# chargen/ALCHEMY

Measured on AMD Instinct MI355X. Metric: ctxt-mul+relinearize/sec at n=2^15, 4 RNS limbs, higher is better.
Workload: dtype u32; 1 GPU; BASELINE config 3: keySwitchQuadCirc(hint, a*b) on linear ciphertexts, n=2^15 (m'=2^16), L=4 primes<2^31, TrivGad hint at the same modulus, CRT-basis in/out, inputs resident in HBM; batch_per_gpu=8192, global_batch=8192, hint=single rank, device_word_bytes=4

## Files before the change

alchemy_amd/csrc/kernel_tensor_split.hpp:

```cpp
#pragma once
#include <hip/hip_runtime.h>
#include "ntt_engine.hpp"

#ifndef ALCH_TI_SPLIT_PASSES
#define ALCH_TI_SPLIT_PASSES 4
#endif

#ifndef ALCH_TI_NT_IN
#define ALCH_TI_NT_IN 0
#endif

#ifndef ALCH_A_PARTIALS
#define ALCH_A_PARTIALS 0
#endif

namespace alch {

template <int LOGN, bool Q30 = false>
__global__ void __launch_bounds__(1 << (LOGN - 6), 4)
k_tensor_intt_split(DevRing<u32> R, const u32* __restrict__ a, const u32* __restrict__ b, int32_t* __restrict__ digits,
                    unsigned nitems, Scal<u32> spre
#if ALCH_A_PARTIALS
                    , const u32* __restrict__ hint, u32* __restrict__ out
#endif
                    ) {
    typedef u32 W;
    constexpr int LOGM = LOGN - 1, M = 1 << LOGM, LT = LOGN - 6, T = 1 << LT;
    typedef Geo<LOGM, LT> G;
    static_assert(G::E == 32 && (LOGM - 2) % 4 == 0, "32 coefficients per lane, stages 4+4+4+2");
    typedef u32 V __attribute__((ext_vector_type(4)));
    typedef int32_t SV __attribute__((ext_vector_type(4)));
    constexpr int NV = G::E / 4;
    extern __shared__ __attribute__((aligned(16))) unsigned char smem[];
    W* lds = reinterpret_cast<W*>(smem);
    const int L = R.L;
    const u32 nct = nitems / (unsigned)L;
    const auto ra = __builtin_amdgcn_make_buffer_rsrc(const_cast<W*>(a), 0, (u32)((size_t)nct * 2 * L * (2 * M) * 4), 0x00020000);
    const auto rb = __builtin_amdgcn_make_buffer_rsrc(const_cast<W*>(b), 0, (u32)((size_t)nct * 2 * L * (2 * M) * 4), 0x00020000);
    const auto rd = __builtin_amdgcn_make_buffer_rsrc(digits, 0, (u32)((size_t)nct * L * (2 * M) * 4), 0x00020000);
    const u32 lane16 = threadIdx.x * 16u;
    constexpr u32 ROW = (u32)(2 * M) * 4u, SLICE = (u32)T * 16u, HALF = (u32)M * 4u;
#if ALCH_A_PARTIALS
    const auto rh = __builtin_amdgcn_make_buffer_rsrc(const_cast<W*>(hint), 0, (u32)((size_t)2 * L * L * (2 * M) * 4), 0x00020000);
    const auto ro = __builtin_amdgcn_make_buffer_rsrc(out, 0, (u32)((size_t)nct * 2 * L * (2 * M) * 4), 0x00020000);
#endif

    for (unsigned item = blockIdx.x; item < nitems; item += gridDim.x) {
        const u32 ct = item / (unsigned)L, i = item % (unsigned)L;
        const ModP<W> m = R.mod[i];
        const W q = m.q, qni = m.qni;
        const W ninv_s = mont_mul(R.ninv_m[i], spre.v[i], m), w1ninv_s = mont_mul(R.w1ninv_m[i], spre.v[i], m);
        const u32 row = ((2 * ct + 1) * (u32)L + i) * ROW;
        const u32 drow = (ct * (u32)L + i) * ROW;
        const int rot = (int)((item ^ (item >> 3)) & (NV - 1));
        const W* twi = R.twi[i];
        V keep[NV];
#pragma unroll 1
        for (int half = 0; half < 2; ++half) {
            int tid = threadIdx.x;
            asm volatile("" : "+v"(tid));
#pragma unroll
            for (int r = 0; r < NV; ++r) {
                const u32 so = row + (u32)half * HALF + SLICE * (u32)((r + rot) & (NV - 1));
                const V va = __builtin_bit_cast(V, __builtin_amdgcn_raw_buffer_load_b128(ra, lane16, so, ALCH_TI_NT_IN));
                const V vb = __builtin_bit_cast(V, __builtin_amdgcn_raw_buffer_load_b128(rb, lane16, so, ALCH_TI_NT_IN));
#if ALCH_A_PARTIALS
                if (out) {
                    const u32 so0 = so - (u32)L * ROW;
                    const u32 piece = (u32)half * HALF + SLICE * (u32)((r + rot) & (NV - 1));
                    const u32 hrow = ((2 * i) * (u32)L + i) * ROW + piece;
                    const V a0v = __builtin_bit_cast(V, __builtin_amdgcn_raw_buffer_load_b128(ra, lane16, so0, ALCH_TI_NT_IN));
                    const V b0v = __builtin_bit_cast(V, __builtin_amdgcn_raw_buffer_load_b128(rb, lane16, so0, ALCH_TI_NT_IN));
                    const V h0v = __builtin_bit_cast(V, __builtin_amdgcn_raw_buffer_load_b128(rh, lane16, hrow, 0));
                    const V h1v = __builtin_bit_cast(V, __builtin_amdgcn_raw_buffer_load_b128(rh, lane16, hrow + (u32)L * ROW, 0));
                    const W sr2 = spre.v[i];
                    V o0v, o1v;
#pragma unroll
                    for (int e = 0; e < 4; ++e) {
                        const W x0 = csub(mont_mul_lazy(a0v[e], sr2, q, qni), q);
                        const W x1 = csub(mont_mul_lazy(va[e], sr2, q, qni), q);
                        const W c2 = csub(mont_mul_lazy(vb[e], x1, q, qni), q);
                        const u64 p0 = (u64)x0 * b0v[e] + (u64)c2 * h0v[e];
                        const u32 m0 = (u32)p0 * qni;
                        o0v[e] = csub((u32)((p0 + (u64)m0 * q) >> 32), q);
                        const u64 p1 = (u64)x0 * vb[e] + (u64)x1 * b0v[e] + (u64)c2 * h1v[e];
                        const u64 p1r = ((u64)csub((W)(p1 >> 32), q) << 32) | (u32)p1;
                        const u32 m1 = (u32)p1r * qni;
                        o1v[e] = csub((u32)((p1r + (u64)m1 * q) >> 32), q);
                    }
                    __builtin_amdgcn_raw_buffer_store_b128(__builtin_bit_cast(decltype(__builtin_amdgcn_raw_buffer_load_b128(ro, 0, 0, 0)), o0v), ro, lane16, so0, 0);
                    ALCH_STORE_GUARD(o0v);
                    __builtin_amdgcn_raw_buffer_store_b128(__builtin_bit_cast(decltype(__builtin_amdgcn_raw_buffer_load_b128(ro, 0, 0, 0)), o1v), ro, lane16, so, 0);
                    ALCH_STORE_GUARD(o1v);
                }
#endif
                V v;
#pragma unroll
                for (int e = 0; e < 4; ++e) v[e] = mont_mul_lazy(va[e], vb[e], q, qni);
                *reinterpret_cast<V*>(&lds[swz<LOGM>((tid + T * ((r + rot) & (NV - 1))) * 4)]) = v;
            }
            lds_barrier();
            NoEpilogue none;
            const int prefix = 2 + half;
#if ALCH_TI_SPLIT_PASSES == 3
            ntt_pass<LOGM, LT, W, 9, 5, true, false, false, W, NoEpilogue&, false, Q30>(lds, twi, q, qni, (W)0, (W)0, tid, prefix, none);
            lds_barrier();
            ntt_pass<LOGM, LT, W, 4, 5, true, false, false, W, NoEpilogue&, false, Q30>(lds, twi, q, qni, (W)0, (W)0, tid, prefix, none);
            lds_barrier();
            ntt_pass<LOGM, LT, W, 0, 4, true, false, false, W, NoEpilogue&, false, Q30>(lds, twi, q, qni, (W)0, (W)0, tid, prefix, none);
            lds_barrier();
#else
            ntt_pass<LOGM, LT, W, 10, 4, true, false, false, W, NoEpilogue&, false, Q30>(lds, twi, q, qni, (W)0, (W)0, tid, prefix, none);
            pair_sync<LOGM>();
            ntt_pass<LOGM, LT, W, 6, 4, true, false, false, W, NoEpilogue&, false, Q30>(lds, twi, q, qni, (W)0, (W)0, tid, prefix, none);
            lds_barrier();
            ntt_pass<LOGM, LT, W, 2, 4, true, false, false, W, NoEpilogue&, false, Q30>(lds, twi, q, qni, (W)0, (W)0, tid, prefix, none);
            lds_barrier();
            ntt_pass<LOGM, LT, W, 0, 2, true, false, false, W, NoEpilogue&, false, Q30>(lds, twi, q, qni, (W)0, (W)0, tid, prefix, none);
            lds_barrier();
#endif
            if (half == 0) {
#pragma unroll
                for (int r = 0; r < NV; ++r) keep[r] = *reinterpret_cast<const V*>(&lds[swz<LOGM>((tid + T * r) * 4)]);
            } else {
                const W hq = (q - 1) >> 1;
#pragma unroll
                for (int r = 0; r < NV; ++r) {
                    const V hi = *reinterpret_cast<const V*>(&lds[swz<LOGM>((tid + T * r) * 4)]);
                    SV z0, z1;
#pragma unroll
                    for (int e = 0; e < 4; ++e) {
                        const W x = csub(keep[r][e], q), y = csub(hi[e], q);
                        const W c0 = csub(mont_mul_lazy((W)(x + y), ninv_s, q, qni), q);
                        const W c1 = csub(mont_mul_lazy((W)(x - y + q), w1ninv_s, q, qni), q);
                        z0[e] = c0 > hq ? (int32_t)c0 - (int32_t)q : (int32_t)c0;
                        z1[e] = c1 > hq ? (int32_t)c1 - (int32_t)q : (int32_t)c1;
                    }
                    const u32 so = drow + SLICE * (u32)r;
                    __builtin_amdgcn_raw_buffer_store_b128(__builtin_bit_cast(decltype(__builtin_amdgcn_raw_buffer_load_b128(rd, 0, 0, 0)), z0), rd, lane16, so, 0);
                    ALCH_STORE_GUARD(z0);
                    __builtin_amdgcn_raw_buffer_store_b128(__builtin_bit_cast(decltype(__builtin_amdgcn_raw_buffer_load_b128(rd, 0, 0, 0)), z1), rd, lane16, so + HALF, 0);
                    ALCH_STORE_GUARD(z1);
                }
            }
            lds_barrier();
        }
    }
}

}
```

alchemy_amd/csrc/ntt_engine.hpp:

```cpp
#pragma once
#include "modarith.hpp"

namespace alch {

template <int LOGN, int LOGT_ = -1>
struct Geo {
    static_assert(LOGN >= 4 && LOGN <= 15, "ring dimension 16 .. 32768 per LDS-resident transform");
    static constexpr int N = 1 << LOGN;
    static constexpr int LOGT = LOGT_ >= 0 ? LOGT_ : ((LOGN - 4 > 10) ? 10 : (LOGN - 4));
    static constexpr int T = 1 << LOGT;
    static constexpr int E = N / T;
    static constexpr int NPASS = (LOGN + 3) / 4;
    static constexpr int NS0 = LOGN - 4 * (NPASS - 1);
    static constexpr bool SWZ = LOGN >= 10;
};

#ifndef ALCH_LDS_PAD
#define ALCH_LDS_PAD 1
#endif
template <int LOGN>
__host__ __device__ constexpr int swz(int idx) {
#if ALCH_LDS_PAD
    return (LOGN >= 10) ? idx + ((idx >> 6) << 2) : idx;
#else
    return (LOGN >= 10) ? (idx ^ (((idx >> 6) & 3) << 2) ^ (((idx >> 8) & 3) << 4)) : idx;
#endif
}
__host__ __device__ constexpr int lds_join(int mapped_base, int mapped_k) {
#if ALCH_LDS_PAD
    return mapped_base + mapped_k;
#else
    return mapped_base ^ mapped_k;
#endif
}
template <int LOGN>
__host__ __device__ constexpr int lds_words() {
#if ALCH_LDS_PAD
    return (LOGN >= 10) ? (1 << LOGN) + (1 << (LOGN - 4)) : (1 << LOGN);
#else
    return 1 << LOGN;
#endif
}

template <typename W> struct Vec4;
template <> struct Vec4<u32> { typedef u32 type __attribute__((ext_vector_type(4))); static constexpr int LANES = 4; };
template <> struct Vec4<u64> { typedef u64 type __attribute__((ext_vector_type(2))); static constexpr int LANES = 2; };

#ifndef ALCH_NO_STORE_GUARD
#define ALCH_STORE_GUARD(v) asm volatile("s_nop 0" ::"v"(v))
#else
#define ALCH_STORE_GUARD(v) ((void)0)
#endif

__device__ __forceinline__ void lds_barrier() {
    asm volatile("s_waitcnt lgkmcnt(0)" ::: "memory");
    __builtin_amdgcn_s_barrier();
    asm volatile("" ::: "memory");
}

template <typename W, int CNT, bool UNIFORM>
__device__ __forceinline__ void load_tw(const W* __restrict__ tw, int first, W (&w)[CNT]) {
    if constexpr (UNIFORM) {
        const int f = __builtin_amdgcn_readfirstlane(first);
#pragma unroll
        for (int c = 0; c < CNT; ++c) w[c] = tw[f + c];
    } else if constexpr (sizeof(W) == 16) {
#pragma unroll
        for (int c = 0; c < CNT; ++c) w[c] = tw[first + c];
    } else if constexpr (sizeof(W) == 4 && CNT >= 4) {
        typedef u32 V __attribute__((ext_vector_type(4)));
#pragma unroll
        for (int c = 0; c < CNT; c += 4) {
            V v = *reinterpret_cast<const V*>(tw + first + c);
#pragma unroll
            for (int e = 0; e < 4; ++e) w[c + e] = v[e];
        }
    } else if constexpr (CNT >= 2) {
        typedef W V __attribute__((ext_vector_type(2)));
#pragma unroll
        for (int c = 0; c < CNT; c += 2) {
            V v = *reinterpret_cast<const V*>(tw + first + c);
            w[c] = v[0];
            w[c + 1] = v[1];
        }
    } else {
        w[0] = tw[first];
    }
}

struct NoEpilogue {
    template <typename W> __device__ __forceinline__ void operator()(int, int, W*) const {}
};

template <int LOGN, int LOGT, typename W, int S0, int NS, bool INVERSE, bool KEEP, bool SERIAL, typename TW, typename Epi,
          bool FOLD = true, bool Q30 = false>
__device__ __forceinline__ void ntt_pass(W* __restrict__ lds, const TW* __restrict__ tw, W q, W qni,
                                         W ninv_m, W w1ninv_m, int t, int prefix, Epi&& epi) {
    typedef Geo<LOGN, LOGT> G;
    constexpr int R = 1 << NS;
    constexpr int LB = LOGN - S0 - NS;
    constexpr int NG = G::E / R;
    static_assert(NG >= 1, "group larger than the per-thread coefficient budget");
    static_assert(NS >= 1 && NS <= 5, "one to five stages per pass");
    typedef typename Vec4<W>::type V;
    constexpr int VL = Vec4<W>::LANES;
    constexpr bool UNIFORM = (LB >= 6) && (G::T >= 64);

#pragma unroll
    for (int g = 0; g < NG; ++g) {
        const int gamma = t + G::T * g;
        const int lo = gamma & ((1 << LB) - 1);
        const int h = gamma >> LB;
        const int base = (h << (NS + LB)) | lo;
        const int sb = swz<LOGN>(base);
        W x[R];
        if constexpr (LB == 0 && R >= VL) {
#pragma unroll
            for (int k = 0; k < R; k += VL) {
                V v = *reinterpret_cast<const V*>(&lds[lds_join(sb, swz<LOGN>(k))]);
#pragma unroll
                for (int e = 0; e < VL; ++e) x[k + e] = v[e];
            }
        } else {
#pragma unroll
            for (int k = 0; k < R; ++k) x[k] = lds[lds_join(sb, swz<LOGN>(k << LB))];
        }
        const int gm = (prefix << S0) + h;
        if constexpr (!INVERSE) {
#pragma unroll
            for (int r = 0; r < NS; ++r) {
                const int half = R >> (r + 1);
                TW w[1 << 4];
                if (r == 0) { TW t1[1]; load_tw<TW, 1, UNIFORM>(tw, gm, t1); w[0] = t1[0]; }
                else if (r == 1) { TW t2[2]; load_tw<TW, 2, UNIFORM>(tw, gm << 1, t2); w[0] = t2[0]; w[1] = t2[1]; }
                else if (r == 2) { TW t4[4]; load_tw<TW, 4, UNIFORM>(tw, gm << 2, t4);
#pragma unroll
                    for (int c = 0; c < 4; ++c) w[c] = t4[c]; }
                else if (r == 3) { TW t8[8]; load_tw<TW, 8, UNIFORM>(tw, gm << 3, t8);
#pragma unroll
                    for (int c = 0; c < 8; ++c) w[c] = t8[c]; }
                else { TW t16[16]; load_tw<TW, 16, UNIFORM>(tw, gm << 4, t16);
#pragma unroll
                    for (int c = 0; c < 16; ++c) w[c] = t16[c]; }
#pragma unroll
                for (int k = 0; k < R; ++k) {
                    if (k & half) continue;
                    if constexpr (Q30) bfly_fwd4(x[k], x[k + half], w[k >> (NS - r)], q, qni);
                    else bfly_fwd_st(x[k], x[k + half], w[k >> (NS - r)], q, qni, r == 0, r == NS - 1);
                }
            }
        } else {
#pragma unroll
            for (int r = NS - 1; r >= 0; --r) {
                const int half = R >> (r + 1);
                TW w[1 << 4];
                if (r == 0) { TW t1[1]; load_tw<TW, 1, UNIFORM>(tw, gm, t1); w[0] = t1[0]; }
                else if (r == 1) { TW t2[2]; load_tw<TW, 2, UNIFORM>(tw, gm << 1, t2); w[0] = t2[0]; w[1] = t2[1]; }
                else if (r == 2) { TW t4[4]; load_tw<TW, 4, UNIFORM>(tw, gm << 2, t4);
#pragma unroll
                    for (int c = 0; c < 4; ++c) w[c] = t4[c]; }
                else if (r == 3) { TW t8[8]; load_tw<TW, 8, UNIFORM>(tw, gm << 3, t8);
#pragma unroll
                    for (int c = 0; c < 8; ++c) w[c] = t8[c]; }
                else { TW t16[16]; load_tw<TW, 16, UNIFORM>(tw, gm << 4, t16);
#pragma unroll
                    for (int c = 0; c < 16; ++c) w[c] = t16[c]; }
#pragma unroll
                for (int k = 0; k < R; ++k) {
                    if (k & half) continue;
                    if (FOLD && S0 == 0 && r == 0) {
                        W a = csub(x[k], q), b = csub(x[k + half], q);
                        x[k] = mont_mul_lazy((W)(a + b), ninv_m, q, qni);
                        x[k + half] = mont_mul_lazy((W)(a - b + q), w1ninv_m, q, qni);
                    } else if constexpr (Q30) {
                        bfly_inv4(x[k], x[k + half], w[k >> (NS - r)], q, qni);
                    } else {
                        bfly_inv(x[k], x[k + half], w[k >> (NS - r)], q, qni);
                    }
                }
            }
        }
        if constexpr (KEEP) {
            epi(g, base, x);
            if constexpr (NG > 1) __builtin_amdgcn_sched_barrier(0);
        } else {
            if constexpr (LB == 0 && R >= VL) {
#pragma unroll
                for (int k = 0; k < R; k += VL) {
                    V v;
#pragma unroll
                    for (int e = 0; e < VL; ++e) v[e] = x[k + e];
                    *reinterpret_cast<V*>(&lds[lds_join(sb, swz<LOGN>(k))]) = v;
                }
            } else {
#pragma unroll
                for (int k = 0; k < R; ++k) lds[lds_join(sb, swz<LOGN>(k << LB))] = x[k];
            }
            if constexpr (NG > 1 && SERIAL) __builtin_amdgcn_sched_barrier(0);
        }
    }
}

#ifndef ALCH_WAVE_LOCAL_PAIR
#define ALCH_WAVE_LOCAL_PAIR 1
#endif
template <int LOGN>
__device__ __forceinline__ void pair_sync() {
    if constexpr (ALCH_WAVE_LOCAL_PAIR && LOGN >= 10) asm volatile("" ::: "memory");
    else lds_barrier();
}

template <int LOGN, typename W, bool KEEP_LAST, bool SERIAL = false, typename TW, typename TWM, typename Epi>
__device__ __forceinline__ void ntt_forward(W* lds, const TW* tw, const TWM* twm, W q, W qni, int tid, Epi&& epi,
                                            int prefix = 1) {
    typedef Geo<LOGN> G;
    constexpr int P = G::NPASS, F = G::NS0, LT = G::LOGT;
    NoEpilogue none;
    if constexpr (P == 1) {
        ntt_pass<LOGN, LT, W, 0, F, false, KEEP_LAST, SERIAL>(lds, twm, q, qni, (W)0, (W)0, tid, prefix, epi);
    } else {
        ntt_pass<LOGN, LT, W, 0, F, false, false, SERIAL>(lds, tw, q, qni, (W)0, (W)0, tid, prefix, none);
        lds_barrier();
        if constexpr (P == 2) {
            ntt_pass<LOGN, LT, W, F, 4, false, KEEP_LAST, SERIAL>(lds, twm, q, qni, (W)0, (W)0, tid, prefix, epi);
        } else {
            ntt_pass<LOGN, LT, W, F, 4, false, false, SERIAL>(lds, tw, q, qni, (W)0, (W)0, tid, prefix, none);
            if constexpr (P == 3) pair_sync<LOGN>(); else lds_barrier();
            if constexpr (P == 3) {
                ntt_pass<LOGN, LT, W, F + 4, 4, false, KEEP_LAST, SERIAL>(lds, twm, q, qni, (W)0, (W)0, tid, prefix, epi);
            } else {
                ntt_pass<LOGN, LT, W, F + 4, 4, false, false, SERIAL>(lds, tw, q, qni, (W)0, (W)0, tid, prefix, none);
                pair_sync<LOGN>();
                ntt_pass<LOGN, LT, W, F + 8, 4, false, KEEP_LAST, SERIAL>(lds, twm, q, qni, (W)0, (W)0, tid, prefix, epi);
            }
        }
    }
    if constexpr (!KEEP_LAST) lds_barrier();
}

struct NoHook { __device__ __forceinline__ void operator()() const {} };

template <int LOGN, typename W, bool KEEP_LAST, bool SERIAL = false, bool FOLD = true, typename TWI, typename Epi, typename Hook = NoHook>
__device__ __forceinline__ void ntt_inverse(W* lds, const TWI* twi, W q, W qni, W ninv_m, W w1ninv_m, int tid,
                                            Epi&& epi, Hook&& hook = NoHook(), int prefix = 1) {
    typedef Geo<LOGN> G;
    constexpr int P = G::NPASS, F = G::NS0, LT = G::LOGT;
    NoEpilogue none;
    constexpr bool U3 = (LOGN - (F + 8) - 4 >= 6), U2 = (LOGN - (F + 4) - 4 >= 6), U1 = (LOGN - F - 4 >= 6);
    bool hooked = false;
    if constexpr (P >= 4) { if (U3 && !hooked) { hook(); hooked = true; }
        ntt_pass<LOGN, LT, W, F + 8, 4, true, false, SERIAL, TWI, NoEpilogue&, FOLD>(lds, twi, q, qni, ninv_m, w1ninv_m, tid, prefix, none); pair_sync<LOGN>(); }
    if constexpr (P >= 3) { if (U2 && !hooked) { hook(); hooked = true; }
        ntt_pass<LOGN, LT, W, F + 4, 4, true, false, SERIAL, TWI, NoEpilogue&, FOLD>(lds, twi, q, qni, ninv_m, w1ninv_m, tid, prefix, none);
        if constexpr (P == 3) pair_sync<LOGN>(); else lds_barrier(); }
    if constexpr (P >= 2) { if (U1 && !hooked) { hook(); hooked = true; }
        ntt_pass<LOGN, LT, W, F, 4, true, false, SERIAL, TWI, NoEpilogue&, FOLD>(lds, twi, q, qni, ninv_m, w1ninv_m, tid, prefix, none); lds_barrier(); }
    if (!hooked) hook();
    ntt_pass<LOGN, LT, W, 0, F, true, KEEP_LAST, SERIAL, TWI, Epi&, FOLD>(lds, twi, q, qni, ninv_m, w1ninv_m, tid, prefix, epi);
    if constexpr (!KEEP_LAST) lds_barrier();
}

}
```

Measured before the change: 555,200 ctxt-mul+relin/s.

## Fold first inverse-NTT stages into load and fuse epilogue into final pass

The tensor+INTT split kernel now applies the first two inverse butterfly stages in registers right after the pointwise product, which cuts the LDS pipeline from 4+4+4+2 stages to three 4-stage passes. The final pass runs with an epilogue lambda that keeps the half-0 results in registers and, on half 1, computes and stores the digits directly, skipping the extra LDS readback. Per-lane twiddle loads are added on load, and digit stores become scalar 32-bit buffer stores instead of 128-bit ones. Separately, uniform twiddle loads are read through the constant address space so the compiler can use scalar loads, at the cost of possible extra register pressure.

```diff
diff --git a/alchemy_amd/csrc/kernel_tensor_split.hpp b/alchemy_amd/csrc/kernel_tensor_split.hpp
--- a/alchemy_amd/csrc/kernel_tensor_split.hpp
+++ b/alchemy_amd/csrc/kernel_tensor_split.hpp
@@ -5,6 +5,11 @@
 #ifndef ALCH_TI_SPLIT_PASSES
 #define ALCH_TI_SPLIT_PASSES 4
 #endif
+#ifndef ALCH_TI_CLOSE_LDS
+#define ALCH_TI_CLOSE_LDS 0
+#endif
+#define ALCH_TI_ONLOAD (ALCH_TI_SPLIT_PASSES == 4)
+#define ALCH_TI_EPI_REGS (ALCH_TI_ONLOAD && !ALCH_TI_CLOSE_LDS)
 
 #ifndef ALCH_TI_NT_IN
 #define ALCH_TI_NT_IN 0
@@ -27,9 +32,11 @@
     typedef u32 W;
     constexpr int LOGM = LOGN - 1, M = 1 << LOGM, LT = LOGN - 6, T = 1 << LT;
     typedef Geo<LOGM, LT> G;
-    static_assert(G::E == 32 && (LOGM - 2) % 4 == 0, "32 coefficients per lane, stages 4+4+4+2");
+    static_assert(G::E == 32 && (LOGM - 2) % 4 == 0, "32 coefficients per lane, stages 2 (on load) + 4 + 4 + 4");
     typedef u32 V __attribute__((ext_vector_type(4)));
+#if !ALCH_TI_EPI_REGS
     typedef int32_t SV __attribute__((ext_vector_type(4)));
+#endif
     constexpr int NV = G::E / 4;
     extern __shared__ __attribute__((aligned(16))) unsigned char smem[];
     W* lds = reinterpret_cast<W*>(smem);
@@ -39,6 +46,9 @@
     const auto rb = __builtin_amdgcn_make_buffer_rsrc(const_cast<W*>(b), 0, (u32)((size_t)nct * 2 * L * (2 * M) * 4), 0x00020000);
     const auto rd = __builtin_amdgcn_make_buffer_rsrc(digits, 0, (u32)((size_t)nct * L * (2 * M) * 4), 0x00020000);
     const u32 lane16 = threadIdx.x * 16u;
+#if ALCH_TI_EPI_REGS
+    const u32 lane4 = threadIdx.x * 4u;
+#endif
     constexpr u32 ROW = (u32)(2 * M) * 4u, SLICE = (u32)T * 16u, HALF = (u32)M * 4u;
 #if ALCH_A_PARTIALS
     const auto rh = __builtin_amdgcn_make_buffer_rsrc(const_cast<W*>(hint), 0, (u32)((size_t)2 * L * L * (2 * M) * 4), 0x00020000);
@@ -54,14 +64,21 @@
         const u32 drow = (ct * (u32)L + i) * ROW;
         const int rot = (int)((item ^ (item >> 3)) & (NV - 1));
         const W* twi = R.twi[i];
-        V keep[NV];
+        W keep[G::E];
 #pragma unroll 1
         for (int half = 0; half < 2; ++half) {
             int tid = threadIdx.x;
             asm volatile("" : "+v"(tid));
+            const int prefix = 2 + half;
 #pragma unroll
             for (int r = 0; r < NV; ++r) {
                 const u32 so = row + (u32)half * HALF + SLICE * (u32)((r + rot) & (NV - 1));
+#if ALCH_TI_ONLOAD
+                const int p = tid + T * ((r + rot) & (NV - 1));
+                typedef W W2 __attribute__((ext_vector_type(2)));
+                const W2 w13 = *reinterpret_cast<const W2*>(twi + (prefix << (LOGM - 1)) + 2 * p);
+                const W w12 = twi[(prefix << (LOGM - 2)) + p];
+#endif
                 const V va = __builtin_bit_cast(V, __builtin_amdgcn_raw_buffer_load_b128(ra, lane16, so, ALCH_TI_NT_IN));
                 const V vb = __builtin_bit_cast(V, __builtin_amdgcn_raw_buffer_load_b128(rb, lane16, so, ALCH_TI_NT_IN));
 #if ALCH_A_PARTIALS
@@ -94,15 +111,54 @@
                     ALCH_STORE_GUARD(o1v);
                 }
 #endif
-                V v;
-#pragma unroll
-                for (int e = 0; e < 4; ++e) v[e] = mont_mul_lazy(va[e], vb[e], q, qni);
+                W c[4];
+#pragma unroll
+                for (int e = 0; e < 4; ++e) c[e] = mont_mul_lazy(va[e], vb[e], q, qni);
+#if ALCH_TI_ONLOAD
+                if constexpr (Q30) {
+                    bfly_inv4(c[0], c[1], w13[0], q, qni); bfly_inv4(c[2], c[3], w13[1], q, qni);
+                    bfly_inv4(c[0], c[2], w12, q, qni);    bfly_inv4(c[1], c[3], w12, q, qni);
+                } else {
+                    bfly_inv(c[0], c[1], (W)w13[0], q, qni);  bfly_inv(c[2], c[3], (W)w13[1], q, qni);
+                    bfly_inv(c[0], c[2], w12, q, qni);        bfly_inv(c[1], c[3], w12, q, qni);
+                }
+#endif
+                const V v = {c[0], c[1], c[2], c[3]};
                 *reinterpret_cast<V*>(&lds[swz<LOGM>((tid + T * ((r + rot) & (NV - 1))) * 4)]) = v;
             }
             lds_barrier();
             NoEpilogue none;
-            const int prefix = 2 + half;
-#if ALCH_TI_SPLIT_PASSES == 3
+            const W hq = (q - 1) >> 1;
+#if ALCH_TI_ONLOAD
+            ntt_pass<LOGM, LT, W, 8, 4, true, false, false, W, NoEpilogue&, false, Q30>(lds, twi, q, qni, (W)0, (W)0, tid, prefix, none);
+            lds_barrier();
+            ntt_pass<LOGM, LT, W, 4, 4, true, false, false, W, NoEpilogue&, false, Q30>(lds, twi, q, qni, (W)0, (W)0, tid, prefix, none);
+            lds_barrier();
+#if ALCH_TI_CLOSE_LDS
+            ntt_pass<LOGM, LT, W, 0, 4, true, false, false, W, NoEpilogue&, false, Q30>(lds, twi, q, qni, (W)0, (W)0, tid, prefix, none);
+            lds_barrier();
+#else
+            auto close = [&](int g, int, W* x) {
+                if (half == 0) {
+#pragma unroll
+                    for (int k = 0; k < 16; ++k) keep[16 * g + k] = x[k];
+                } else {
+#pragma unroll
+                    for (int k = 0; k < 16; ++k) {
+                        const W u = csub(keep[16 * g + k], q), y = csub(x[k], q);
+                        const W c0 = csub(mont_mul_lazy((W)(u + y), ninv_s, q, qni), q);
+                        const W c1 = csub(mont_mul_lazy((W)(u - y + q), w1ninv_s, q, qni), q);
+                        const int32_t z0 = c0 > hq ? (int32_t)c0 - (int32_t)q : (int32_t)c0;
+                        const int32_t z1 = c1 > hq ? (int32_t)c1 - (int32_t)q : (int32_t)c1;
+                        const u32 so = drow + 4u * (u32)(T * g + (k << (LOGM - 4)));
+                        __builtin_amdgcn_raw_buffer_store_b32(z0, rd, lane4, so, 0);
+                        __builtin_amdgcn_raw_buffer_store_b32(z1, rd, lane4, so + HALF, 0);
+                    }
+                }
+            };
+            ntt_pass<LOGM, LT, W, 0, 4, true, true, false, W, decltype(close)&, false, Q30>(lds, twi, q, qni, (W)0, (W)0, tid, prefix, close);
+#endif
+#elif ALCH_TI_SPLIT_PASSES == 3
             ntt_pass<LOGM, LT, W, 9, 5, true, false, false, W, NoEpilogue&, false, Q30>(lds, twi, q, qni, (W)0, (W)0, tid, prefix, none);
             lds_barrier();
             ntt_pass<LOGM, LT, W, 4, 5, true, false, false, W, NoEpilogue&, false, Q30>(lds, twi, q, qni, (W)0, (W)0, tid, prefix, none);
@@ -119,18 +175,22 @@
             ntt_pass<LOGM, LT, W, 0, 2, true, false, false, W, NoEpilogue&, false, Q30>(lds, twi, q, qni, (W)0, (W)0, tid, prefix, none);
             lds_barrier();
 #endif
+#if !ALCH_TI_EPI_REGS
             if (half == 0) {
 #pragma unroll
-                for (int r = 0; r < NV; ++r) keep[r] = *reinterpret_cast<const V*>(&lds[swz<LOGM>((tid + T * r) * 4)]);
+                for (int r = 0; r < NV; ++r) {
+                    const V lo = *reinterpret_cast<const V*>(&lds[swz<LOGM>((tid + T * r) * 4)]);
+#pragma unroll
+                    for (int e = 0; e < 4; ++e) keep[4 * r + e] = lo[e];
+                }
             } else {
-                const W hq = (q - 1) >> 1;
 #pragma unroll
                 for (int r = 0; r < NV; ++r) {
                     const V hi = *reinterpret_cast<const V*>(&lds[swz<LOGM>((tid + T * r) * 4)]);
                     SV z0, z1;
 #pragma unroll
                     for (int e = 0; e < 4; ++e) {
-                        const W x = csub(keep[r][e], q), y = csub(hi[e], q);
+                        const W x = csub(keep[4 * r + e], q), y = csub(hi[e], q);
                         const W c0 = csub(mont_mul_lazy((W)(x + y), ninv_s, q, qni), q);
                         const W c1 = csub(mont_mul_lazy((W)(x - y + q), w1ninv_s, q, qni), q);
                         z0[e] = c0 > hq ? (int32_t)c0 - (int32_t)q : (int32_t)c0;
@@ -143,6 +203,7 @@
                     ALCH_STORE_GUARD(z1);
                 }
             }
+#endif
             lds_barrier();
         }
     }
diff --git a/alchemy_amd/csrc/ntt_engine.hpp b/alchemy_amd/csrc/ntt_engine.hpp
--- a/alchemy_amd/csrc/ntt_engine.hpp
+++ b/alchemy_amd/csrc/ntt_engine.hpp
@@ -58,10 +58,21 @@
     asm volatile("" ::: "memory");
 }
 
+#ifndef ALCH_TW_CONSTANT_AS
+#define ALCH_TW_CONSTANT_AS 1
+#endif
 template <typename W, int CNT, bool UNIFORM>
 __device__ __forceinline__ void load_tw(const W* __restrict__ tw, int first, W (&w)[CNT]) {
     if constexpr (UNIFORM) {
         const int f = __builtin_amdgcn_readfirstlane(first);
+#if defined(__HIP_DEVICE_COMPILE__) && ALCH_TW_CONSTANT_AS
+        if constexpr (sizeof(W) <= 8) {
+            const __attribute__((address_space(4))) W* ct = (const __attribute__((address_space(4))) W*)(tw + f);
+#pragma unroll
+            for (int c = 0; c < CNT; ++c) w[c] = ct[c];
+            return;
+        }
+#endif
 #pragma unroll
         for (int c = 0; c < CNT; ++c) w[c] = tw[f + c];
     } else if constexpr (sizeof(W) == 16) {
```

Measured after the change: 566,000 ctxt-mul+relin/s, median of 6. +2.0%, better.
